# UoB-HPC/stdpar-nbody

Measured on AMD Instinct MI355X. Metric: body-steps/sec + %FP64 peak, 3D double all-pairs N=2^20 at 1/2/4/8 GPUs, higher is better.
Workload: dtype f64

## Files before the change

### stdpar-nbody_amd/csrc/all_pairs.hip

```cpp
#include "common.hpp"

#include <atomic>
#include <cstdlib>
#include <mutex>
#include <type_traits>
#include <vector>

namespace nbody {

constexpr int kBlock = 256;
constexpr int kWaves = kBlock / 64;

struct ap_config {
  int split = 0;
  int tpt   = 0;
  int path  = 0;
};
static std::atomic<uint32_t> g_ap_default{0};

static ap_config ap_config_of(const nbody_state* s) {
  const uint32_t t = s->tuning ? s->tuning : g_ap_default.load(std::memory_order_relaxed);
  ap_config c;
  c.split = int(t & 15u);
  c.tpt   = int((t >> 4) & 3u);
// ... 14 lines not shown
__global__ __launch_bounds__(kBlock) void all_pairs_softened_kernel(const T* __restrict__ m, const T* __restrict__ x,
                                                                    T* __restrict__ a, T c, uint32_t sz, uint32_t first,
                                                                    uint32_t count, T e2) {
  const k1_rule* const rule = nullptr;
#define K1_SOFT true
#include "k1_tile_body.inc"
#undef K1_SOFT
}

template <typename T, int D>
__global__ __launch_bounds__(kBlock) void pack_sources_kernel(const T* __restrict__ m, const T* __restrict__ x,
                                                              src_rec<T, D>* __restrict__ out, uint32_t sz, uint32_t padded) {
  const uint32_t j = blockIdx.x * kBlock + threadIdx.x;
  if (j >= padded) return;
  src_rec<T, D> r;
#pragma unroll
  for (int k = 0; k < 3; ++k) r.p[k] = (k < D && j < sz) ? x[uint64_t(j) * D + (k < D ? k : 0)] : T(0);
  r.m    = j < sz ? m[j] : T(0);
  out[j] = r;
}

template <typename T, int D, bool PACK, bool MOMENTS>
__global__ __launch_bounds__(kBlock) void k1_prepare_kernel(const T* __restrict__ m, const T* __restrict__ x, src_rec<T, D>* __restrict__ out,
                                                            uint32_t sz, uint32_t padded, k1_rule* rule, double* partial,
                                                            uint32_t* turn, uint32_t turn_words) {
  const uint32_t j = blockIdx.x * kBlock + threadIdx.x;
  T p[D];
#pragma unroll
  for (int k = 0; k < D; ++k) p[k] = j < sz ? x[uint64_t(j) * D + k] : T(0);
  if constexpr (PACK) {
    if (j < padded) {
      src_rec<T, D> r;
#pragma unroll
      for (int k = 0; k < 3; ++k) r.p[k] = k < D ? p[k < D ? k : 0] : T(0);
      r.m    = j < sz ? m[j] : T(0);
      out[j] = r;
    }
  }
  __shared__ double red[2 * D][kWaves];
  __shared__ bool last_s;
  const int lane = threadIdx.x & 63, wave = threadIdx.x >> 6;
  if constexpr (MOMENTS) {
    double s1[D], s2[D];
#pragma unroll
    for (int k = 0; k < D; ++k) {
      const double d = j < sz ? double(p[k]) - double(x[k]) : 0.0;
      s1[k] = d;
      s2[k] = d * d;
    }
#pragma unroll
    for (int k = 0; k < D; ++k)
      for (int off = 32; off > 0; off >>= 1) {
        s1[k] += __shfl_xor(s1[k], off, 64);
        s2[k] += __shfl_xor(s2[k], off, 64);
      }
    if (lane == 0) {
#pragma unroll
      for (int k = 0; k < D; ++k) {
        red[k][wave]     = s1[k];
// ... 52 lines not shown
  for (uint32_t w = threadIdx.x; w < turn_words; w += kBlock) turn[w] = 0u;
  if (threadIdx.x == 0) __hip_atomic_store(&rule->ticket, 0u, __ATOMIC_RELAXED, __HIP_MEMORY_SCOPE_AGENT);
}

template <int JS>
constexpr int kSgprWaves = JS > kWaves ? JS : kWaves;

constexpr uint32_t kTurnSpins  = 1u << 26;
constexpr uint32_t kTurnPoison = 0xffffffffu;
struct k1_status {
  uint32_t err, block, group, chunk;
  unsigned long long polls, waits;
};
struct k1_handoff {
  void* sums;
  uint32_t* turn;
  k1_status* status;
  uint32_t spins;
  uint32_t delay;
  uint32_t late;
};
template <typename T, int D, int R, int JS, int RULE = 0>
__global__ __launch_bounds__(64 * kSgprWaves<JS>) void all_pairs_force_sgpr_kernel(const src_rec<T, D>* __restrict__ packed,
                                                                                   const T* __restrict__ x, T* a, T c, uint32_t sz,
                                                                                   uint32_t first, uint32_t count,
                                                                                   uint32_t tiles_per_chunk, k1_handoff h,
                                                                                   const k1_rule* __restrict__ rule) {
  [[maybe_unused]] constexpr T e2 = T(0);
#define K1_SOFT false
#include "k1_sgpr_body.inc"
#undef K1_SOFT
}
template <typename T, int D, int R, int JS>
__global__ __launch_bounds__(64 * kSgprWaves<JS>) void all_pairs_softened_sgpr_kernel(const src_rec<T, D>* __restrict__ packed,
                                                                                      const T* __restrict__ x, T* a, T c, uint32_t sz,
                                                                                      uint32_t first, uint32_t count,
                                                                                      uint32_t tiles_per_chunk, k1_handoff h, T e2) {
  constexpr int RULE = 0;
  const k1_rule* const rule = nullptr;
#define K1_SOFT true
#include "k1_sgpr_body.inc"
#undef K1_SOFT
}

namespace {
struct scratch_buf {
  void* ptr  = nullptr;
  size_t cap = 0;
};
struct packed_slot {
  int device;
  hipStream_t stream;
  scratch_buf buf[6];
  std::vector<void*> retired;
  bool k1_dirty  = false;
  bool k1_failed = false;
};
std::mutex g_packed_mu;
std::vector<packed_slot> g_packed_slots;
}

int ap_scratch_get(hipStream_t st, int which, size_t bytes, void** out) {
  const int dev = stream_device(st);
  std::lock_guard<std::mutex> lock(g_packed_mu);
  packed_slot* slot = nullptr;
  for (auto& sl : g_packed_slots)
    if (sl.stream == st && sl.device == dev) slot = &sl;
  if (slot && slot->buf[which].cap >= bytes) {
    *out = slot->buf[which].ptr;
    return NBODY_OK;
  }
  hipStreamCaptureStatus cs = hipStreamCaptureStatusNone;
  if (st != nullptr) (void)hipStreamIsCapturing(st, &cs);
  if (cs != hipStreamCaptureStatusNone) {
    set_error("all-pairs: the scratch buffers of this stream must exist before a step is recorded "
              "(call nbody_all_pairs_force once outside nbody_graph_begin/end, or use a context from nbody_create)");
// ... 78 lines not shown
    else p.r = blocks_r2 * uint64_t(p.js) >= 8192 ? 2 : 1;
  }
  *out = p;
  return NBODY_OK;
}

int ap_pack_sources(const nbody_state* s, hipStream_t st, void** packed_out) {
  const uint32_t padded = (s->sz + kTileJ - 1) / kTileJ * kTileJ;
  const size_t tsz      = s->dtype == NBODY_F32 ? 4 : 8;
  void* scratch         = nullptr;
  if (int r = ap_scratch_get(st, 0, 4 * tsz * size_t(padded), &scratch)) return r;
  int rc = dispatch(s->dtype, s->dim, [&](auto tg) {
    using T         = typename decltype(tg)::type;
    constexpr int D = decltype(tg)::dim;
    hipLaunchKernelGGL((pack_sources_kernel<T, D>), dim3((padded + kBlock - 1) / kBlock), dim3(kBlock), 0, st,
                       static_cast<const T*>(s->m), static_cast<const T*>(s->x), static_cast<src_rec<T, D>*>(scratch), s->sz, padded);
    NB_HIP(hipGetLastError());
    return int(NBODY_OK);
  });
  *packed_out = scratch;
  return rc;
}

static size_t ap_rule_bytes(uint32_t sz, int dim) {
  const size_t padded = (size_t(sz) + kTileJ - 1) / kTileJ * kTileJ;
  return 32 + sizeof(double) * 2 * size_t(dim) * (padded / kBlock);
}

template <typename T, int D>
static int ap_prepare(const nbody_state* s, hipStream_t st, bool pack, src_rec<T, D>** packed_out, const k1_rule** rule_out,
                      uint32_t* turn, size_t turn_words, bool with_rule = true) {
  const uint32_t padded = (s->sz + kTileJ - 1) / kTileJ * kTileJ;
  const bool moments    = with_rule && s->sz >= kFarMinBodies;
  void* scratch         = nullptr;
  if (pack)
    if (int r = ap_scratch_get(st, 0, 4 * sizeof(T) * size_t(padded), &scratch)) return r;
  void* q = nullptr;
  if (int r = ap_scratch_get(st, 3, ap_rule_bytes(s->sz, D), &q)) return r;
  auto* rule    = static_cast<k1_rule*>(q);
  auto* partial = reinterpret_cast<double*>(static_cast<char*>(q) + 32);
  auto* out     = static_cast<src_rec<T, D>*>(scratch);
  const dim3 grid(padded / kBlock), block(kBlock);
  const T *m = static_cast<const T*>(s->m), *x = static_cast<const T*>(s->x);
  const uint32_t words = uint32_t(turn_words);
  if (pack && moments) hipLaunchKernelGGL((k1_prepare_kernel<T, D, true, true>), grid, block, 0, st, m, x, out, s->sz, padded, rule, partial, turn, words);
  else if (pack) hipLaunchKernelGGL((k1_prepare_kernel<T, D, true, false>), grid, block, 0, st, m, x, out, s->sz, padded, rule, partial, turn, words);
  else if (moments) hipLaunchKernelGGL((k1_prepare_kernel<T, D, false, true>), grid, block, 0, st, m, x, out, s->sz, padded, rule, partial, turn, words);
  NB_HIP(hipGetLastError());
  if (packed_out) *packed_out = out;
  *rule_out = moments ? rule : nullptr;
  return NBODY_OK;
}

constexpr uint32_t kCollectMaxBlocks = 2048;
static bool k1_collect(uint32_t target_blocks, uint32_t chunks) {
  uint32_t limit = kCollectMaxBlocks;
  if (const char* e = experiment_env("NBODY_K1_COLLECT_MAX")) limit = uint32_t(atoi(e));
  return chunks > 1 && uint64_t(target_blocks) * chunks <= limit;
}
template <typename T, int D, int R, int JS>
static size_t k1_collect_bytes(uint32_t target_blocks, uint32_t chunks) {
  constexpr int TG = kSgprWaves<JS> / JS;
  return sizeof(T) * size_t(chunks) * target_blocks * TG * R * D * 64;
}

template <int R, int JS>
static size_t sgpr_turn_words(uint32_t count) {
  constexpr int TG = kSgprWaves<JS> / JS, TB = TG * 64 * R;
  return size_t((count + TB - 1) / TB) * TG;
}

template <typename T, int D, int R, int JS, bool SOFT>
static int launch_all_pairs_sgpr(const nbody_state* s, const k1_plan& plan, hipStream_t st, T e2) {
  constexpr int TB = (kSgprWaves<JS> / JS) * 64 * R;
  uint32_t blocks  = (s->count + TB - 1) / TB;
  if (blocks == 0) return NBODY_OK;
  k1_handoff h{nullptr, nullptr, nullptr, kTurnSpins, 0u, 0u};
  if (plan.chunks > 1) {
    void* q = nullptr;
    if (int r = ap_scratch_get(st, 1, sizeof(uint32_t) * sgpr_turn_words<R, JS>(s->count), &q)) return r;
    h.turn = static_cast<uint32_t*>(q);
    if (k1_collect(blocks, plan.chunks)) {
      if (int r = ap_scratch_get(st, 5, k1_collect_bytes<T, D, R, JS>(blocks, plan.chunks), &q)) return r;
      h.sums = q;
    }
    if (int r = ap_scratch_get(st, 4, sizeof(k1_status), &q)) return r;
    h.status = static_cast<k1_status*>(q);
    if (const char* e = experiment_env("NBODY_K1_TURN_SPINS")) h.spins = uint32_t(strtoul(e, nullptr, 10));
    if (const char* e = experiment_env("NBODY_K1_HANDOFF_DELAY")) h.delay = uint32_t(strtoul(e, nullptr, 10));
    if (const char* e = experiment_env("NBODY_K1_HANDOFF_LATE")) h.late = uint32_t(strtoul(e, nullptr, 10));
    if (const char* e = experiment_env("NBODY_K1_NO_HANDOFF"); e && e[0] == '1') h.turn = nullptr, h.sums = nullptr;
    if (const char* e = experiment_env("NBODY_K1_COLLECT"); e && e[0] == '0') h.sums = nullptr;
  }
  src_rec<T, D>* packed = nullptr;
  const k1_rule* rule   = nullptr;
  if (int r = ap_prepare<T, D>(s, st, true, &packed, &rule, h.turn, h.turn ? sgpr_turn_words<R, JS>(s->count) : 0, !SOFT)) return r;
  if constexpr (SOFT) {
    hipLaunchKernelGGL((all_pairs_softened_sgpr_kernel<T, D, R, JS>), dim3(blocks, plan.chunks), dim3(64 * kSgprWaves<JS>), 0, st,
                       packed, static_cast<const T*>(s->x), static_cast<T*>(s->a), static_cast<T>(s->c), s->sz, s->first, s->count,
                       plan.tiles_per_chunk, h, e2);
    NB_HIP(hipGetLastError());
    if (h.turn != nullptr && h.sums == nullptr) ap_status_mark(st);
    return NBODY_OK;
  }
#ifdef NBODY_EXPERIMENTS
  if (const char* e = getenv("NBODY_K1_RULE_FORCE"); e && JS == 8 && D == 3) {
    if (e[0] == '1')
      hipLaunchKernelGGL((all_pairs_force_sgpr_kernel<T, D, R, JS, 1>), dim3(blocks, plan.chunks), dim3(64 * kSgprWaves<JS>), 0, st,
                         packed, static_cast<const T*>(s->x), static_cast<T*>(s->a), static_cast<T>(s->c), s->sz, s->first, s->count,
                         plan.tiles_per_chunk, h, rule);
    else
      hipLaunchKernelGGL((all_pairs_force_sgpr_kernel<T, D, R, JS, 2>), dim3(blocks, plan.chunks), dim3(64 * kSgprWaves<JS>), 0, st,
                         packed, static_cast<const T*>(s->x), static_cast<T*>(s->a), static_cast<T>(s->c), s->sz, s->first, s->count,
                         plan.tiles_per_chunk, h, rule);
    NB_HIP(hipGetLastError());
    return NBODY_OK;
  }
#endif
  hipLaunchKernelGGL((all_pairs_force_sgpr_kernel<T, D, R, JS>), dim3(blocks, plan.chunks), dim3(64 * kSgprWaves<JS>), 0, st,
                     packed, static_cast<const T*>(s->x), static_cast<T*>(s->a), static_cast<T>(s->c), s->sz, s->first, s->count,
                     plan.tiles_per_chunk, h, rule);
  NB_HIP(hipGetLastError());
  if (h.turn != nullptr && h.sums == nullptr) ap_status_mark(st);
  return NBODY_OK;
}

template <typename T, int D, int R, int JS, bool SOFT>
static int launch_all_pairs(const nbody_state* s, hipStream_t st, T e2) {
  constexpr int TB = (kWaves / JS) * 64 * R;
  uint32_t blocks  = (s->count + TB - 1) / TB;
  if (blocks == 0) return NBODY_OK;
  if constexpr (SOFT) {
    hipLaunchKernelGGL((all_pairs_softened_kernel<T, D, R, JS>), dim3(blocks), dim3(kBlock), 0, st, static_cast<const T*>(s->m),
                       static_cast<const T*>(s->x), static_cast<T*>(s->a), static_cast<T>(s->c), s->sz, s->first, s->count, e2);
    NB_HIP(hipGetLastError());
    return NBODY_OK;
  }
  const k1_rule* rule = nullptr;
  if (int r = ap_prepare<T, D>(s, st, false, nullptr, &rule, nullptr, 0)) return r;
  hipLaunchKernelGGL((all_pairs_force_kernel<T, D, R, JS>), dim3(blocks), dim3(kBlock), 0, st, static_cast<const T*>(s->m),
                     static_cast<const T*>(s->x), static_cast<T*>(s->a), static_cast<T>(s->c), s->sz, s->first, s->count, rule);
  NB_HIP(hipGetLastError());
  return NBODY_OK;
}

template <typename F>
static bool with_k1_instance(const k1_plan& p, F&& fn) {
#define NB_CASE(RR, JJ)                                                                       \
  if (p.r == RR && p.js == JJ) {                                                              \
    fn(std::integral_constant<int, RR>{}, std::integral_constant<int, JJ>{});                 \
    return true;                                                                              \
  }
  NB_CASE(1, 1);
  NB_CASE(1, 2);
  NB_CASE(1, 4);
  NB_CASE(2, 1);
  NB_CASE(2, 2);
  NB_CASE(2, 4);
  if (p.scalar) {
    NB_CASE(1, 8);
    NB_CASE(2, 8);
  }
// ... 4 lines not shown
template <typename T, int D, bool SOFT = false>
static int all_pairs_dispatch(const nbody_state* s, hipStream_t st, T e2 = T(0)) {
  k1_plan p;
  if (int rc = plan_all_pairs<T>(s, &p)) return rc;
  int rc = NBODY_OK;
  const bool found = with_k1_instance(p, [&](auto r, auto js) {
    constexpr int R = decltype(r)::value, JS = decltype(js)::value;
    rc = p.scalar ? launch_all_pairs_sgpr<T, D, R, JS, SOFT>(s, p, st, e2)
                  : (JS <= kWaves ? launch_all_pairs<T, D, R, (JS <= kWaves ? JS : 1), SOFT>(s, st, e2) : int(NBODY_ERR_ARG));
  });
  if (!found) {
    set_error("all-pairs: unsupported config split=%d targets_per_thread=%d", p.js, p.r);
    return NBODY_ERR_ARG;
  }
  return rc;
}

template <typename T, int D>
static int all_pairs_describe(const nbody_state* s, char* out, size_t len) {
  k1_plan p;
  if (int rc = plan_all_pairs<T>(s, &p)) return rc;
  const char* t = sizeof(T) == 8 ? "double" : "float";
  const char* pair = sizeof(T) == 4 ? (s->sz >= kFarMinBodies ? "rsq+rcp[m y^3 at r2 >= 4 if sparse]" : "rsq+rcp")
                                    : s->sz >= kFarMinBodies ? "far3[-eps if sparse]/near3" : "far3/near3";
  if (p.scalar) {
    bool collect = false;
    with_k1_instance(p, [&](auto r, auto js) {
      constexpr int TB = (kSgprWaves<decltype(js)::value> / decltype(js)::value) * 64 * decltype(r)::value;
      collect = k1_collect((s->count + TB - 1) / TB, p.chunks);
    });
    snprintf(out, len, "all_pairs_force_sgpr_kernel<%s,%d,R=%d,JS=%d> tile=%d chunks=%u%s pair=%s", t, D, p.r, p.js, kTileJ, p.chunks,
             p.chunks > 1 ? (collect ? "(summed in chunk order by the last to arrive)" : "(summed in turn into a)") : "", pair);
  }
  else
    snprintf(out, len, "all_pairs_force_kernel<%s,%d,R=%d,JS=%d> tile=%d chunks=1 pair=%s", t, D, p.r, p.js, kTileJ, pair);
  return NBODY_OK;
}

int ap_scratch_reserve(hipStream_t st, const nbody_state* s) {
  void* q             = nullptr;
  const size_t tsz    = s->dtype == NBODY_F32 ? 4 : 8;
  const size_t padded = (size_t(s->sz) + 2 * kTileJ - 1) / (2 * kTileJ) * (2 * kTileJ);
  if (int r = ap_scratch_get(st, 0, 4 * tsz * padded, &q)) return r;
  if (int r = ap_scratch_get(st, 3, ap_rule_bytes(s->sz, s->dim), &q)) return r;
  return dispatch(s->dtype, s->dim, [&](auto tg) {
    using T = typename decltype(tg)::type;
    k1_plan p;
    if (int rc = plan_all_pairs<T>(s, &p)) return rc;
    if (!p.scalar || p.chunks <= 1) return int(NBODY_OK);
    size_t words = 0;
    with_k1_instance(p, [&](auto r, auto js) { words = sgpr_turn_words<decltype(r)::value, decltype(js)::value>(s->count); });
    if (!words) return int(NBODY_OK);
    if (int rc = ap_scratch_get(st, 1, sizeof(uint32_t) * words, &q)) return rc;
    size_t sums = 0;
    with_k1_instance(p, [&](auto r, auto js) {
      constexpr int RR = decltype(r)::value, JJ = decltype(js)::value;
      const uint32_t blocks = (s->count + (kSgprWaves<JJ> / JJ) * 64 * RR - 1) / ((kSgprWaves<JJ> / JJ) * 64 * RR);
      if (k1_collect(blocks, p.chunks)) sums = k1_collect_bytes<T, decltype(tg)::dim, RR, JJ>(blocks, p.chunks);
    });
    if (sums)
      if (int rc = ap_scratch_get(st, 5, sums, &q)) return rc;
    return ap_scratch_get(st, 4, sizeof(k1_status), &q);
  });
}

void ap_status_mark(hipStream_t st) {
// ... 590 lines not shown
  }
  return NBODY_OK;
}

extern "C" int nbody_all_pairs_describe(const nbody_state* s, char* out, size_t len) {
  NB_ARG(out != nullptr && len > 0, "out is NULL");
  if (int r = check_state(s)) return r;
  return dispatch(s->dtype, s->dim, [&](auto tg) {
    using TG = decltype(tg);
    return all_pairs_describe<typename TG::type, TG::dim>(s, out, len);
  });
}

extern "C" int nbody_all_pairs_pair_rule(const nbody_state* s, void* stream, int* sparse_out, double* volume_out) {
  NB_ARG(sparse_out != nullptr, "sparse_out is NULL");
  if (int r = check_state(s)) return r;
  device_guard guard(stream_device(as_stream(stream)));
  *sparse_out = 0;
  if (volume_out) *volume_out = 0.0;
  return dispatch(s->dtype, s->dim, [&](auto tg) {
    using T         = typename decltype(tg)::type;
    constexpr int D = decltype(tg)::dim;
    const k1_rule* rule = nullptr;
    if (int r = ap_prepare<T, D>(s, as_stream(stream), false, nullptr, &rule, nullptr, 0)) return r;
    if (rule == nullptr) return int(NBODY_OK);
    k1_rule host;
    NB_HIP(hipMemcpyAsync(&host, rule, sizeof host, hipMemcpyDeviceToHost, as_stream(stream)));
    NB_HIP(hipStreamSynchronize(as_stream(stream)));
    *sparse_out = host.sparse ? 1 : 0;
    if (volume_out) *volume_out = host.volume;
    return int(NBODY_OK);
  });
}

extern "C" int nbody_all_pairs_force(const nbody_state* s, void* stream) {
  if (int r = check_state(s)) return r;
  device_guard guard(stream_device(as_stream(stream)));
  return dispatch(s->dtype, s->dim, [&](auto tg) {
    using TG = decltype(tg);
    return all_pairs_dispatch<typename TG::type, TG::dim>(s, as_stream(stream));
  });
}

extern "C" int nbody_all_pairs_softened_force(const nbody_state* s, double eps, void* stream) {
  if (int r = check_state(s)) return r;
  return dispatch(s->dtype, s->dim, [&](auto tg) {
    using TG = decltype(tg);
// ... 35 lines not shown
```

### stdpar-nbody_amd/csrc/common.hpp

```cpp
#pragma once
#include <hip/hip_runtime.h>

#include <cfloat>
#include <cstdarg>
#include <cstdint>
#include <cstdio>
#include <cstdlib>
#include <cstring>

#include "../../include/nbody_hip.h"

namespace nbody {

void set_error(const char* fmt, ...);
int hip_fail(hipError_t e, const char* what, const char* file, int line);

#define NB_HIP(call)                                                                   \
  do {                                                                                 \
    hipError_t e_ = (call);                                                            \
    if (e_ != hipSuccess) return ::nbody::hip_fail(e_, #call, __FILE__, __LINE__);     \
  } while (0)

#define NB_ARG(cond, ...)                \
  do {                                   \
// ... 111 lines not shown
    if constexpr (POLISH >= 3) {
      double q = __builtin_fma(e2, e2, e2);
      return __builtin_fma(zm, q, zm);
    } else {
      return __builtin_fma(zm, e2, zm);
    }
  }

  static constexpr uint32_t near_hi = 0x3EF00000u;
  static constexpr uint32_t far_hi = 0x40100000u;
  template <bool EPS = true>
  __device__ static __forceinline__ double weight_far(double r2, double mj, double k15, double k1875, double eps = DBL_EPSILON) {
    double y  = __builtin_amdgcn_rsq(r2);
    double a  = y * y;
    double e  = __builtin_fma(-r2, a, 1.0);
    double y3 = a * y;
    double p  = __builtin_fma(e, k1875, k15);
    double g;
    if constexpr (EPS) g = __builtin_fma(p, e, -(eps * y3));
    else g = p * e;
    double my = mj * y3;
    return __builtin_fma(my, g, my);
  }
};

template <>
struct pair_math<float> {
  static constexpr float tiny = 1e-37f;
  __device__ static __forceinline__ float weight(float r2, float mj) {
    float y0 = __builtin_amdgcn_rsqf(r2);
    float d3 = __builtin_fmaf(r2, r2 * y0, FLT_EPSILON);
    return __builtin_amdgcn_rcpf(d3) * mj;
  }
  static constexpr uint32_t far_bits = 0x40800000u;
};

template <typename T, int D>
struct alignas(sizeof(T) * 4) src_rec {
  T p[3];
  T m;
};

template <typename T, int D>
__device__ __forceinline__ void pair_accumulate(T (&acc)[D], const T (&xi)[D], const src_rec<T, D>& s) {
  T d[D];
#pragma unroll
  for (int k = 0; k < D; ++k) d[k] = s.p[k] - xi[k];
  T r2 = pair_math<T>::tiny;
#pragma unroll
  for (int k = 0; k < D; ++k) r2 = __builtin_elementwise_fma(d[k], d[k], r2);
  T w = pair_math<T>::weight(r2, s.m);
#pragma unroll
  for (int k = 0; k < D; ++k) acc[k] = __builtin_elementwise_fma(w, d[k], acc[k]);
}

template <typename T, int D, int NB>
__device__ __forceinline__ void pair_accumulate_multi(T (&acc)[D], const T (&xi)[D], const src_rec<T, D>* s) {
  T d[NB][D], r2[NB], w[NB];
#pragma unroll
  for (int b = 0; b < NB; ++b) {
#pragma unroll
    for (int k = 0; k < D; ++k) d[b][k] = s[b].p[k] - xi[k];
  }
#pragma unroll
  for (int b = 0; b < NB; ++b) {
// ... 25 lines not shown
#pragma unroll
    for (int k = 0; k < D; ++k) r2[b] = __builtin_elementwise_fma(d[b][k], d[b][k], r2[b]);
  }
#pragma unroll
  for (int b = 0; b < NB; ++b) {
    w[b]              = pair_math<double>::weight_far(r2[b], s[b].m, k15, k1875);
    const uint32_t hi = uint32_t(__builtin_bit_cast(unsigned long long, r2[b]) >> 32);
    lowest            = hi < lowest ? hi : lowest;
  }
#pragma unroll
  for (int b = 0; b < NB; ++b) {
#pragma unroll
    for (int k = 0; k < D; ++k) acc[k] = __builtin_elementwise_fma(w[b], d[b][k], acc[k]);
  }
}

template <typename T>
struct pair_consts {
  __device__ __forceinline__ pair_consts() {}
};
template <>
struct pair_consts<double> {
  double k15, k1875;
  __device__ __forceinline__ pair_consts() : k15(1.5), k1875(1.875) {
    asm volatile("" : "+v"(k15));
    asm volatile("" : "+s"(k1875));
  }
};

template <typename T, int D, int R, int U, bool ffar>
__device__ __forceinline__ void pair_batch(T (&acc)[R][D], const T (&xi)[R][D], const src_rec<T, D> (&s)[U],
                                           const pair_consts<T>& pc) {
  if constexpr (sizeof(T) == 4) {
    if constexpr (!ffar) {
#pragma unroll
      for (int u = 0; u < U; ++u)
#pragma unroll
        for (int r = 0; r < R; ++r) pair_accumulate<T, D>(acc[r], xi[r], s[u]);
    } else {
      T d[U][R][D], r2[U][R], w[U][R];
      uint32_t lowest = 0xffffffffu;
#pragma unroll
      for (int u = 0; u < U; ++u)
#pragma unroll
        for (int r = 0; r < R; ++r) {
#pragma unroll
          for (int k = 0; k < D; ++k) d[u][r][k] = s[u].p[k] - xi[r][k];
          T q = pair_math<T>::tiny;
#pragma unroll
          for (int k = 0; k < D; ++k) q = __builtin_elementwise_fma(d[u][r][k], d[u][r][k], q);
          r2[u][r]            = q;
          const uint32_t bits = __builtin_bit_cast(uint32_t, q);
          lowest              = bits < lowest ? bits : lowest;
        }
      T y[U][R];
// ... 21 lines not shown
#pragma unroll
          for (int k = 0; k < D; ++k) acc[r][k] = __builtin_elementwise_fma(w[u][r], d[u][r][k], acc[r][k]);
    }
  } else {
    T d[U][R][D], r2[U][R], w[U][R];
    uint32_t lowest = 0xffffffffu;
#pragma unroll
    for (int u = 0; u < U; ++u)
#pragma unroll
      for (int r = 0; r < R; ++r) {
#pragma unroll
        for (int k = 0; k < D; ++k) d[u][r][k] = s[u].p[k] - xi[r][k];
        T q = pair_math<T>::tiny;
#pragma unroll
        for (int k = 0; k < D; ++k) q = __builtin_elementwise_fma(d[u][r][k], d[u][r][k], q);
        r2[u][r] = q;
        const uint32_t hi = uint32_t(__builtin_bit_cast(unsigned long long, q) >> 32);
        lowest            = hi < lowest ? hi : lowest;
      }
    if constexpr (!ffar) {
#pragma unroll
      for (int u = 0; u < U; ++u)
#pragma unroll
        for (int r = 0; r < R; ++r) w[u][r] = pair_math<T>::template weight_far<true>(r2[u][r], s[u].m, pc.k15, pc.k1875);
      if (__builtin_expect(__builtin_amdgcn_ballot_w64(lowest < pair_math<T>::near_hi) != 0ull, 0)) {
#pragma unroll
        for (int u = 0; u < U; ++u)
#pragma unroll
          for (int r = 0; r < R; ++r) {
            const uint32_t hi = uint32_t(__builtin_bit_cast(unsigned long long, r2[u][r]) >> 32);
            const T wn        = pair_math<T>::template weight<3>(r2[u][r], s[u].m);
            w[u][r]           = hi < pair_math<T>::near_hi ? wn : w[u][r];
          }
      }
    } else if (__builtin_expect(__builtin_amdgcn_ballot_w64(lowest < pair_math<T>::far_hi) == 0ull, 1)) {
#pragma unroll
      for (int u = 0; u < U; ++u)
#pragma unroll
        for (int r = 0; r < R; ++r) w[u][r] = pair_math<T>::template weight_far<false>(r2[u][r], s[u].m, pc.k15, pc.k1875);
    } else {
#pragma unroll
      for (int u = 0; u < U; ++u)
#pragma unroll
        for (int r = 0; r < R; ++r) {
          const uint32_t hi  = uint32_t(__builtin_bit_cast(unsigned long long, r2[u][r]) >> 32);
          const uint32_t ehi = hi < pair_math<T>::far_hi ? 0x3CB00000u : 0u;
          const T eps        = __builtin_bit_cast(T, (unsigned long long)ehi << 32);
          w[u][r]            = pair_math<T>::template weight_far<true>(r2[u][r], s[u].m, pc.k15, pc.k1875, eps);
        }
      if (__builtin_expect(__builtin_amdgcn_ballot_w64(lowest < pair_math<T>::near_hi) != 0ull, 0)) {
#pragma unroll
        for (int u = 0; u < U; ++u)
#pragma unroll
          for (int r = 0; r < R; ++r) {
            const uint32_t hi = uint32_t(__builtin_bit_cast(unsigned long long, r2[u][r]) >> 32);
            const T wn        = pair_math<T>::template weight<3>(r2[u][r], s[u].m);
            w[u][r]           = hi < pair_math<T>::near_hi ? wn : w[u][r];
          }
      }
    }
#pragma unroll
    for (int u = 0; u < U; ++u)
#pragma unroll
      for (int r = 0; r < R; ++r)
#pragma unroll
        for (int k = 0; k < D; ++k) acc[r][k] = __builtin_elementwise_fma(w[u][r], d[u][r][k], acc[r][k]);
  }
}

template <typename T>
__device__ __forceinline__ T soft_weight(T q, T mj, const pair_consts<T>& pc) {
  if constexpr (sizeof(T) == 8) {
    return pair_math<double>::template weight_far<false>(q, mj, pc.k15, pc.k1875);
  } else {
    const T y = __builtin_amdgcn_rsqf(q);
    return mj * ((y * y) * y);
  }
}

template <typename T, int D, int R, int U>
__device__ __forceinline__ void pair_batch_soft(T (&acc)[R][D], const T (&xi)[R][D], const src_rec<T, D> (&s)[U],
                                                const pair_consts<T>& pc, T e2) {
  T d[U][R][D], q[U][R], w[U][R];
#pragma unroll
  for (int u = 0; u < U; ++u)
#pragma unroll
    for (int r = 0; r < R; ++r) {
#pragma unroll
      for (int k = 0; k < D; ++k) d[u][r][k] = s[u].p[k] - xi[r][k];
      T t = e2;
#pragma unroll
      for (int k = 0; k < D; ++k) t = __builtin_elementwise_fma(d[u][r][k], d[u][r][k], t);
      q[u][r] = t;
    }
#pragma unroll
  for (int u = 0; u < U; ++u)
#pragma unroll
    for (int r = 0; r < R; ++r) w[u][r] = soft_weight<T>(q[u][r], s[u].m, pc);
#pragma unroll
  for (int u = 0; u < U; ++u)
#pragma unroll
    for (int r = 0; r < R; ++r)
#pragma unroll
      for (int k = 0; k < D; ++k) acc[r][k] = __builtin_elementwise_fma(w[u][r], d[u][r][k], acc[r][k]);
}

template <typename T>
constexpr T kSoftMinE2 = sizeof(T) == 4 ? T(0x1p-84f) : T(0x1p-680);

template <typename T>
inline int check_softening(double eps, T* e2_out) {
  NB_ARG(eps > 0.0 && eps <= DBL_MAX, "softening length eps = %g must be finite and > 0", eps);
  const T te = T(eps);
  const T e2 = te * te;
  NB_ARG(e2 >= kSoftMinE2<T> && e2 <= (sizeof(T) == 4 ? T(FLT_MAX) : T(DBL_MAX)),
         "softening length eps = %g: eps^2 = %g in %s is outside [%g, max]: its square must be a normal number whose ^(-3/2) is finite",
         eps, double(e2), sizeof(T) == 4 ? "float" : "double", double(kSoftMinE2<T>));
  *e2_out = e2;
  return NBODY_OK;
}

// ... 6 lines not shown
};
constexpr uint32_t kFarMinBodies = 32768;
template <int D>
constexpr double kFarMinVolume = D == 3 ? 1.7e5 : 6.4e4;
__device__ __forceinline__ bool ap_far_mode(const k1_rule* __restrict__ rule) {
  if (rule == nullptr) return false;
  return __builtin_amdgcn_readfirstlane(int(rule->sparse)) != 0;
}

constexpr int kTileJ = 512;

typedef uint32_t sgpr16 __attribute__((ext_vector_type(16)));
template <typename V>
__device__ __forceinline__ sgpr16 sload16(const void* p, V& tie) {
  sgpr16 r;
  asm volatile("s_load_dwordx16 %0, %2, 0x0" : "=s"(r), "+v"(tie) : "s"(p));
  return r;
}
template <typename V>
__device__ __forceinline__ void swait(sgpr16& v, V& tie) {
  asm volatile("s_waitcnt lgkmcnt(0)" : "+s"(v), "+v"(tie));
}

inline int check_tuning(int split, int tpt, int path) {
  NB_ARG(split == 0 || split == 1 || split == 2 || split == 4 || split == 8, "split must be 0, 1, 2, 4 or 8 (got %d)", split);
  NB_ARG(tpt >= 0 && tpt <= 2, "targets_per_thread must be 0, 1 or 2 (got %d)", tpt);
  NB_ARG(path >= 0 && path <= 2, "source path must be 0 (auto), 1 (LDS tiles) or 2 (scalar stream), got %d", path);
  return NBODY_OK;
}

int ap_scratch_reserve(hipStream_t st, const nbody_state* view);
void ap_scratch_release(hipStream_t st);
int ap_scratch_get(hipStream_t st, int which, size_t bytes, void** out);
void ap_status_mark(hipStream_t st);
int ap_status_read(hipStream_t st, unsigned long long out[6], bool clear);
int ap_pack_sources(const nbody_state* s, hipStream_t st, void** packed_out);
void ap_auto_chunks(uint32_t sz, uint32_t* chunks, uint32_t* tiles_per_chunk);
int energies_from_sums(const nbody_state* s, hipStream_t st, int (*fill)(void* sums, void* ctx), void* ctx, void* ke_out, void* pe_out);

}
```

### stdpar-nbody_amd/csrc/k1_sgpr_body.inc

```
  using rec_t = src_rec<T, D>;
  constexpr int TG  = kSgprWaves<JS> / JS;
  constexpr int TB  = TG * 64 * R;
  constexpr int SUB = kTileJ / JS;
  __shared__ T partial[(JS > 1) ? (JS - 1) * TG * 64 * R * D : 1];
  const int lane   = threadIdx.x & 63;
  const int wave   = __builtin_amdgcn_readfirstlane(threadIdx.x >> 6);
  const int tgroup = wave / JS;
  const int jpart  = wave % JS;
  T xi[R][D], acc[R][D];
  uint32_t ti[R];
#pragma unroll
  for (int r = 0; r < R; ++r) {
    uint32_t local = blockIdx.x * TB + tgroup * (64 * R) + r * 64 + lane;
    ti[r]          = local;
    uint64_t i     = uint64_t(first) + (local < count ? local : 0u);
#pragma unroll
    for (int k = 0; k < D; ++k) {
      xi[r][k]  = x[i * D + k];
      acc[r][k] = T(0);
    }
  }
  const uint32_t ntiles = (sz + kTileJ - 1) / kTileJ;
  const uint32_t t0     = blockIdx.y * tiles_per_chunk;
  const uint32_t t1     = min(ntiles, t0 + tiles_per_chunk);
  const pair_consts<T> pc;
  const bool ffar       = !K1_SOFT && ap_far_mode(rule);
  const uint32_t nsteps = (t1 - t0) * SUB;
  constexpr int U = 64 / int(sizeof(rec_t));
  struct batch_t {
    rec_t r[U];
  };
  auto batch = [&](uint32_t k) { return packed + (uint64_t(t0 + k / SUB) * kTileJ + uint32_t(jpart) * SUB + (k % SUB)); };
  auto run = [&](auto ff) {
    constexpr bool FF = decltype(ff)::value;
    sgpr16 A = sload16(batch(0), xi[0][0]), B;
    for (uint32_t k = 0; k < nsteps; k += 2 * U) {
      swait(A, acc[0][0]);
      B = sload16(batch(k + U), xi[0][0]);
      {
        const batch_t ba = __builtin_bit_cast(batch_t, A);
        if constexpr (K1_SOFT) pair_batch_soft<T, D, R, U>(acc, xi, ba.r, pc, e2);
        else pair_batch<T, D, R, U, FF>(acc, xi, ba.r, pc);
      }
      swait(B, acc[0][0]);
      A = sload16(batch(k + 2 * U < nsteps ? k + 2 * U : k), xi[0][0]);
      {
        const batch_t bb = __builtin_bit_cast(batch_t, B);
        if constexpr (K1_SOFT) pair_batch_soft<T, D, R, U>(acc, xi, bb.r, pc, e2);
        else pair_batch<T, D, R, U, FF>(acc, xi, bb.r, pc);
      }
    }
    swait(A, acc[0][0]);
  };
  if constexpr (K1_SOFT) run(std::false_type{});
  else if constexpr (RULE == 1) run(std::false_type{});
  else if constexpr (RULE == 2) run(std::true_type{});
  else if (ffar) run(std::true_type{});
  else run(std::false_type{});
  if constexpr (JS > 1) {
    if (jpart > 0) {
#pragma unroll
      for (int r = 0; r < R; ++r)
#pragma unroll
        for (int k = 0; k < D; ++k) partial[((((jpart - 1) * TG + tgroup) * R + r) * D + k) * 64 + lane] = acc[r][k];
    }
    __syncthreads();
    if (jpart == 0) {
#pragma unroll
      for (int p = 1; p < JS; ++p)
#pragma unroll
        for (int r = 0; r < R; ++r)
#pragma unroll
          for (int k = 0; k < D; ++k) acc[r][k] += partial[((((p - 1) * TG + tgroup) * R + r) * D + k) * 64 + lane];
    }
  }
// ... 118 lines not shown
```

### stdpar-nbody_amd/csrc/k1_tile_body.inc

```
  using rec_t = src_rec<T, D>;
  constexpr int TG  = kWaves / JS;
  constexpr int TB  = TG * 64 * R;
  constexpr int LPT = kTileJ / kBlock;
  constexpr int SUB = kTileJ / JS;

  __shared__ rec_t tile[kTileJ];
  __shared__ T partial[(JS > 1) ? (JS - 1) * TG * 64 * R * D : 1];

  const int lane   = threadIdx.x & 63;
  const int wave   = threadIdx.x >> 6;
  const int tgroup = wave / JS;
  const int jpart  = wave % JS;

  T xi[R][D], acc[R][D];
  uint32_t ti[R];
#pragma unroll
  for (int r = 0; r < R; ++r) {
    uint32_t local = blockIdx.x * TB + tgroup * (64 * R) + r * 64 + lane;
    ti[r]          = local;
    uint64_t i     = uint64_t(first) + (local < count ? local : 0u);
#pragma unroll
    for (int k = 0; k < D; ++k) {
      xi[r][k]  = x[i * D + k];
      acc[r][k] = T(0);
// ... 17 lines not shown
#pragma unroll
        for (int k = 0; k < D; ++k) stage[q].p[k] = T(0);
        stage[q].m = T(0);
      }
      if (D == 2) stage[q].p[2] = T(0);
    }
  };

  stage_load(0);
  auto run = [&](auto ff) {
    constexpr bool FF = decltype(ff)::value;
    for (uint32_t t = 0; t < ntiles; ++t) {
      __syncthreads();
#pragma unroll
      for (int q = 0; q < LPT; ++q) tile[q * kBlock + threadIdx.x] = stage[q];
      __syncthreads();
      if (t + 1 < ntiles) stage_load(t + 1);

      const rec_t* src = &tile[jpart * SUB];
      constexpr int U  = 64 / int(sizeof(rec_t));
#pragma unroll 2
      for (int jj = 0; jj < SUB; jj += U) {
        rec_t s[U];
#pragma unroll
        for (int u = 0; u < U; ++u) s[u] = src[jj + u];
        if constexpr (K1_SOFT) pair_batch_soft<T, D, R, U>(acc, xi, s, pc, e2);
        else pair_batch<T, D, R, U, FF>(acc, xi, s, pc);
      }
    }
  };
  if constexpr (K1_SOFT) run(std::false_type{});
  else if (ffar) run(std::true_type{});
  else run(std::false_type{});

  if constexpr (JS > 1) {
    __syncthreads();
    if (jpart > 0) {
#pragma unroll
      for (int r = 0; r < R; ++r)
#pragma unroll
        for (int k = 0; k < D; ++k) partial[((((jpart - 1) * TG + tgroup) * R + r) * D + k) * 64 + lane] = acc[r][k];
    }
    __syncthreads();
    if (jpart == 0) {
#pragma unroll
      for (int p = 1; p < JS; ++p)
#pragma unroll
        for (int r = 0; r < R; ++r)
#pragma unroll
          for (int k = 0; k < D; ++k) acc[r][k] += partial[((((p - 1) * TG + tgroup) * R + r) * D + k) * 64 + lane];
// ... 12 lines not shown
```

Measured before the change: 1.739 million.

## Precompute per-source 1.5m and 1.875m constants to fold the far-field weight polynomial

The f64 prepare kernel now writes per-source constants 1.5*m and 1.875*m into a new scratch buffer. The SGPR force kernel streams these alongside the packed sources, splitting them across a vector global load and a scalar load. It then uses a folded weight formula (t = fma(e, m1875, m15); s = fma(t, e, m)) that drops the per-pair multiplies by mass. This cuts FP64 VALU ops per interaction, at the cost of extra memory traffic, extra scratch, and a more complex load/wait pipeline that adds VGPR pressure.

```diff
diff --git a/stdpar-nbody_amd/csrc/all_pairs.hip b/stdpar-nbody_amd/csrc/all_pairs.hip
--- a/stdpar-nbody_amd/csrc/all_pairs.hip
+++ b/stdpar-nbody_amd/csrc/all_pairs.hip
@@ -60,7 +60,7 @@
 
 template <typename T, int D, bool PACK, bool MOMENTS>
 __global__ __launch_bounds__(kBlock) void k1_prepare_kernel(const T* __restrict__ m, const T* __restrict__ x, src_rec<T, D>* __restrict__ out,
-                                                            uint32_t sz, uint32_t padded, k1_rule* rule, double* partial,
+                                                            cst_batch* __restrict__ cst, uint32_t sz, uint32_t padded, k1_rule* rule, double* partial,
                                                             uint32_t* turn, uint32_t turn_words) {
   const uint32_t j = blockIdx.x * kBlock + threadIdx.x;
   T p[D];
@@ -73,6 +73,11 @@
       for (int k = 0; k < 3; ++k) r.p[k] = k < D ? p[k < D ? k : 0] : T(0);
       r.m    = j < sz ? m[j] : T(0);
       out[j] = r;
+      if constexpr (sizeof(T) == 8) {
+        const src_cst<T> k  = src_cst<T>::of(r.m);
+        cst[j / 2].m15[j % 2]   = k.m15;
+        cst[j / 2].m1875[j % 2] = k.m1875;
+      }
     }
   }
   __shared__ double red[2 * D][kWaves];
@@ -171,6 +176,7 @@
 };
 template <typename T, int D, int R, int JS, int RULE = 0>
 __global__ __launch_bounds__(64 * kSgprWaves<JS>) void all_pairs_force_sgpr_kernel(const src_rec<T, D>* __restrict__ packed,
+                                                                                   const cst_batch* __restrict__ cst,
                                                                                    const T* __restrict__ x, T* a, T c, uint32_t sz,
                                                                                    uint32_t first, uint32_t count,
                                                                                    uint32_t tiles_per_chunk, k1_handoff h,
@@ -182,6 +188,7 @@
 }
 template <typename T, int D, int R, int JS>
 __global__ __launch_bounds__(64 * kSgprWaves<JS>) void all_pairs_softened_sgpr_kernel(const src_rec<T, D>* __restrict__ packed,
+                                                                                      const cst_batch* __restrict__ cst,
                                                                                       const T* __restrict__ x, T* a, T c, uint32_t sz,
                                                                                       uint32_t first, uint32_t count,
                                                                                       uint32_t tiles_per_chunk, k1_handoff h, T e2) {
@@ -200,7 +207,7 @@
 struct packed_slot {
   int device;
   hipStream_t stream;
-  scratch_buf buf[6];
+  scratch_buf buf[7];
   std::vector<void*> retired;
   bool k1_dirty  = false;
   bool k1_failed = false;
@@ -325,32 +332,40 @@
   return rc;
 }
 
+static size_t ap_cst_bytes(size_t padded) { return sizeof(cst_batch) * (padded / 2); }
+
 static size_t ap_rule_bytes(uint32_t sz, int dim) {
   const size_t padded = (size_t(sz) + kTileJ - 1) / kTileJ * kTileJ;
   return 32 + sizeof(double) * 2 * size_t(dim) * (padded / kBlock);
 }
 
 template <typename T, int D>
-static int ap_prepare(const nbody_state* s, hipStream_t st, bool pack, src_rec<T, D>** packed_out, const k1_rule** rule_out,
-                      uint32_t* turn, size_t turn_words, bool with_rule = true) {
+static int ap_prepare(const nbody_state* s, hipStream_t st, bool pack, src_rec<T, D>** packed_out, const cst_batch** cst_out,
+                      const k1_rule** rule_out, uint32_t* turn, size_t turn_words, bool with_rule = true) {
   const uint32_t padded = (s->sz + kTileJ - 1) / kTileJ * kTileJ;
   const bool moments    = with_rule && s->sz >= kFarMinBodies;
   void* scratch         = nullptr;
-  if (pack)
+  void* consts          = nullptr;
+  if (pack) {
     if (int r = ap_scratch_get(st, 0, 4 * sizeof(T) * size_t(padded), &scratch)) return r;
+    if (sizeof(T) == 8)
+      if (int r = ap_scratch_get(st, 6, ap_cst_bytes(padded), &consts)) return r;
+  }
   void* q = nullptr;
   if (int r = ap_scratch_get(st, 3, ap_rule_bytes(s->sz, D), &q)) return r;
   auto* rule    = static_cast<k1_rule*>(q);
   auto* partial = reinterpret_cast<double*>(static_cast<char*>(q) + 32);
   auto* out     = static_cast<src_rec<T, D>*>(scratch);
+  auto* cst     = static_cast<cst_batch*>(consts);
   const dim3 grid(padded / kBlock), block(kBlock);
   const T *m = static_cast<const T*>(s->m), *x = static_cast<const T*>(s->x);
   const uint32_t words = uint32_t(turn_words);
-  if (pack && moments) hipLaunchKernelGGL((k1_prepare_kernel<T, D, true, true>), grid, block, 0, st, m, x, out, s->sz, padded, rule, partial, turn, words);
-  else if (pack) hipLaunchKernelGGL((k1_prepare_kernel<T, D, true, false>), grid, block, 0, st, m, x, out, s->sz, padded, rule, partial, turn, words);
-  else if (moments) hipLaunchKernelGGL((k1_prepare_kernel<T, D, false, true>), grid, block, 0, st, m, x, out, s->sz, padded, rule, partial, turn, words);
+  if (pack && moments) hipLaunchKernelGGL((k1_prepare_kernel<T, D, true, true>), grid, block, 0, st, m, x, out, cst, s->sz, padded, rule, partial, turn, words);
+  else if (pack) hipLaunchKernelGGL((k1_prepare_kernel<T, D, true, false>), grid, block, 0, st, m, x, out, cst, s->sz, padded, rule, partial, turn, words);
+  else if (moments) hipLaunchKernelGGL((k1_prepare_kernel<T, D, false, true>), grid, block, 0, st, m, x, out, cst, s->sz, padded, rule, partial, turn, words);
   NB_HIP(hipGetLastError());
   if (packed_out) *packed_out = out;
+  if (cst_out) *cst_out = cst;
   *rule_out = moments ? rule : nullptr;
   return NBODY_OK;
 }
@@ -396,11 +411,12 @@
     if (const char* e = experiment_env("NBODY_K1_COLLECT"); e && e[0] == '0') h.sums = nullptr;
   }
   src_rec<T, D>* packed = nullptr;
+  const cst_batch* cst  = nullptr;
   const k1_rule* rule   = nullptr;
-  if (int r = ap_prepare<T, D>(s, st, true, &packed, &rule, h.turn, h.turn ? sgpr_turn_words<R, JS>(s->count) : 0, !SOFT)) return r;
+  if (int r = ap_prepare<T, D>(s, st, true, &packed, &cst, &rule, h.turn, h.turn ? sgpr_turn_words<R, JS>(s->count) : 0, !SOFT)) return r;
   if constexpr (SOFT) {
     hipLaunchKernelGGL((all_pairs_softened_sgpr_kernel<T, D, R, JS>), dim3(blocks, plan.chunks), dim3(64 * kSgprWaves<JS>), 0, st,
-                       packed, static_cast<const T*>(s->x), static_cast<T*>(s->a), static_cast<T>(s->c), s->sz, s->first, s->count,
+                       packed, cst, static_cast<const T*>(s->x), static_cast<T*>(s->a), static_cast<T>(s->c), s->sz, s->first, s->count,
                        plan.tiles_per_chunk, h, e2);
     NB_HIP(hipGetLastError());
     if (h.turn != nullptr && h.sums == nullptr) ap_status_mark(st);
@@ -410,18 +426,18 @@
   if (const char* e = getenv("NBODY_K1_RULE_FORCE"); e && JS == 8 && D == 3) {
     if (e[0] == '1')
       hipLaunchKernelGGL((all_pairs_force_sgpr_kernel<T, D, R, JS, 1>), dim3(blocks, plan.chunks), dim3(64 * kSgprWaves<JS>), 0, st,
-                         packed, static_cast<const T*>(s->x), static_cast<T*>(s->a), static_cast<T>(s->c), s->sz, s->first, s->count,
+                         packed, cst, static_cast<const T*>(s->x), static_cast<T*>(s->a), static_cast<T>(s->c), s->sz, s->first, s->count,
                          plan.tiles_per_chunk, h, rule);
     else
       hipLaunchKernelGGL((all_pairs_force_sgpr_kernel<T, D, R, JS, 2>), dim3(blocks, plan.chunks), dim3(64 * kSgprWaves<JS>), 0, st,
-                         packed, static_cast<const T*>(s->x), static_cast<T*>(s->a), static_cast<T>(s->c), s->sz, s->first, s->count,
+                         packed, cst, static_cast<const T*>(s->x), static_cast<T*>(s->a), static_cast<T>(s->c), s->sz, s->first, s->count,
                          plan.tiles_per_chunk, h, rule);
     NB_HIP(hipGetLastError());
     return NBODY_OK;
   }
 #endif
   hipLaunchKernelGGL((all_pairs_force_sgpr_kernel<T, D, R, JS>), dim3(blocks, plan.chunks), dim3(64 * kSgprWaves<JS>), 0, st,
-                     packed, static_cast<const T*>(s->x), static_cast<T*>(s->a), static_cast<T>(s->c), s->sz, s->first, s->count,
+                     packed, cst, static_cast<const T*>(s->x), static_cast<T*>(s->a), static_cast<T>(s->c), s->sz, s->first, s->count,
                      plan.tiles_per_chunk, h, rule);
   NB_HIP(hipGetLastError());
   if (h.turn != nullptr && h.sums == nullptr) ap_status_mark(st);
@@ -440,7 +456,7 @@
     return NBODY_OK;
   }
   const k1_rule* rule = nullptr;
-  if (int r = ap_prepare<T, D>(s, st, false, nullptr, &rule, nullptr, 0)) return r;
+  if (int r = ap_prepare<T, D>(s, st, false, nullptr, nullptr, &rule, nullptr, 0)) return r;
   hipLaunchKernelGGL((all_pairs_force_kernel<T, D, R, JS>), dim3(blocks), dim3(kBlock), 0, st, static_cast<const T*>(s->m),
                      static_cast<const T*>(s->x), static_cast<T*>(s->a), static_cast<T>(s->c), s->sz, s->first, s->count, rule);
   NB_HIP(hipGetLastError());
@@ -491,7 +507,7 @@
   if (int rc = plan_all_pairs<T>(s, &p)) return rc;
   const char* t = sizeof(T) == 8 ? "double" : "float";
   const char* pair = sizeof(T) == 4 ? (s->sz >= kFarMinBodies ? "rsq+rcp[m y^3 at r2 >= 4 if sparse]" : "rsq+rcp")
-                                    : s->sz >= kFarMinBodies ? "far3[-eps if sparse]/near3" : "far3/near3";
+                                    : s->sz >= kFarMinBodies ? "far3m[-eps if sparse]/near3" : "far3m/near3";
   if (p.scalar) {
     bool collect = false;
     with_k1_instance(p, [&](auto r, auto js) {
@@ -511,6 +527,8 @@
   const size_t tsz    = s->dtype == NBODY_F32 ? 4 : 8;
   const size_t padded = (size_t(s->sz) + 2 * kTileJ - 1) / (2 * kTileJ) * (2 * kTileJ);
   if (int r = ap_scratch_get(st, 0, 4 * tsz * padded, &q)) return r;
+  if (s->dtype == NBODY_F64)
+    if (int r = ap_scratch_get(st, 6, ap_cst_bytes(padded), &q)) return r;
   if (int r = ap_scratch_get(st, 3, ap_rule_bytes(s->sz, s->dim), &q)) return r;
   return dispatch(s->dtype, s->dim, [&](auto tg) {
     using T = typename decltype(tg)::type;
@@ -1147,7 +1165,7 @@
     using T         = typename decltype(tg)::type;
     constexpr int D = decltype(tg)::dim;
     const k1_rule* rule = nullptr;
-    if (int r = ap_prepare<T, D>(s, as_stream(stream), false, nullptr, &rule, nullptr, 0)) return r;
+    if (int r = ap_prepare<T, D>(s, as_stream(stream), false, nullptr, nullptr, &rule, nullptr, 0)) return r;
     if (rule == nullptr) return int(NBODY_OK);
     k1_rule host;
     NB_HIP(hipMemcpyAsync(&host, rule, sizeof host, hipMemcpyDeviceToHost, as_stream(stream)));
diff --git a/stdpar-nbody_amd/csrc/common.hpp b/stdpar-nbody_amd/csrc/common.hpp
--- a/stdpar-nbody_amd/csrc/common.hpp
+++ b/stdpar-nbody_amd/csrc/common.hpp
@@ -157,6 +157,21 @@
     double my = mj * y3;
     return __builtin_fma(my, g, my);
   }
+
+  static constexpr double eps23 = 2.0 / 3.0 * DBL_EPSILON;
+  template <bool EPS, bool SMASS = false>
+  __device__ static __forceinline__ double weight_far_folded(double r2, double mj, double m15, double m1875, double keps = eps23) {
+    double y  = __builtin_amdgcn_rsq(r2);
+    double a  = y * y;
+    double e  = __builtin_fma(-r2, a, 1.0);
+    double y3 = a * y;
+    if constexpr (EPS) e = __builtin_fma(-keps, y3, e);
+    double t = __builtin_fma(e, m1875, m15);
+    double s;
+    if constexpr (SMASS) asm("v_fma_f64 %0, %1, %2, %3" : "=v"(s) : "v"(t), "v"(e), "s"(mj));
+    else s = __builtin_fma(t, e, mj);
+    return y3 * s;
+  }
 };
 
 template <>
@@ -176,6 +191,19 @@
   T m;
 };
 
+template <typename T>
+struct src_cst {
+  __device__ __forceinline__ static src_cst of(T) { return {}; }
+};
+template <>
+struct src_cst<double> {
+  double m15, m1875;
+  __device__ __forceinline__ static src_cst of(double m) { return {1.5 * m, 1.875 * m}; }
+};
+struct alignas(32) cst_batch {
+  double m15[2], m1875[2];
+};
+
 template <typename T, int D>
 __device__ __forceinline__ void pair_accumulate(T (&acc)[D], const T (&xi)[D], const src_rec<T, D>& s) {
   T d[D];
@@ -247,15 +275,17 @@
 template <>
 struct pair_consts<double> {
   double k15, k1875;
-  __device__ __forceinline__ pair_consts() : k15(1.5), k1875(1.875) {
+  double keps;
+  __device__ __forceinline__ pair_consts() : k15(1.5), k1875(1.875), keps(pair_math<double>::eps23) {
     asm volatile("" : "+v"(k15));
     asm volatile("" : "+s"(k1875));
+    asm("" : "+s"(keps));
   }
 };
 
 template <typename T, int D, int R, int U, bool ffar>
 __device__ __forceinline__ void pair_batch(T (&acc)[R][D], const T (&xi)[R][D], const src_rec<T, D> (&s)[U],
-                                           const pair_consts<T>& pc) {
+                                           const src_cst<T> (&kc)[U], const pair_consts<T>& pc) {
   if constexpr (sizeof(T) == 4) {
     if constexpr (!ffar) {
 #pragma unroll
@@ -323,7 +353,8 @@
 #pragma unroll
       for (int u = 0; u < U; ++u)
 #pragma unroll
-        for (int r = 0; r < R; ++r) w[u][r] = pair_math<T>::template weight_far<true>(r2[u][r], s[u].m, pc.k15, pc.k1875);
+        for (int r = 0; r < R; ++r)
+          w[u][r] = pair_math<T>::template weight_far_folded<true>(r2[u][r], s[u].m, kc[u].m15, kc[u].m1875, pc.keps);
       if (__builtin_expect(__builtin_amdgcn_ballot_w64(lowest < pair_math<T>::near_hi) != 0ull, 0)) {
 #pragma unroll
         for (int u = 0; u < U; ++u)
@@ -338,16 +369,15 @@
 #pragma unroll
       for (int u = 0; u < U; ++u)
 #pragma unroll
-        for (int r = 0; r < R; ++r) w[u][r] = pair_math<T>::template weight_far<false>(r2[u][r], s[u].m, pc.k15, pc.k1875);
+        for (int r = 0; r < R; ++r) w[u][r] = pair_math<T>::template weight_far_folded<false>(r2[u][r], s[u].m, kc[u].m15, kc[u].m1875);
     } else {
 #pragma unroll
       for (int u = 0; u < U; ++u)
 #pragma unroll
         for (int r = 0; r < R; ++r) {
-          const uint32_t hi  = uint32_t(__builtin_bit_cast(unsigned long long, r2[u][r]) >> 32);
-          const uint32_t ehi = hi < pair_math<T>::far_hi ? 0x3CB00000u : 0u;
-          const T eps        = __builtin_bit_cast(T, (unsigned long long)ehi << 32);
-          w[u][r]            = pair_math<T>::template weight_far<true>(r2[u][r], s[u].m, pc.k15, pc.k1875, eps);
+          const uint32_t hi = uint32_t(__builtin_bit_cast(unsigned long long, r2[u][r]) >> 32);
+          const T mine      = hi < pair_math<T>::far_hi ? pc.keps : T(0);
+          w[u][r]           = pair_math<T>::template weight_far_folded<true>(r2[u][r], s[u].m, kc[u].m15, kc[u].m1875, mine);
         }
       if (__builtin_expect(__builtin_amdgcn_ballot_w64(lowest < pair_math<T>::near_hi) != 0ull, 0)) {
 #pragma unroll
@@ -369,6 +399,13 @@
   }
 }
 
+template <typename T, int D, int R, int U, bool ffar>
+__device__ __forceinline__ void pair_batch(T (&acc)[R][D], const T (&xi)[R][D], const src_rec<T, D> (&s)[U], const pair_consts<T>& pc) {
+  static_assert(sizeof(T) == 4, "f64 callers pass the sources' constants (src_cst)");
+  const src_cst<T> none[U] = {};
+  pair_batch<T, D, R, U, ffar>(acc, xi, s, none, pc);
+}
+
 template <typename T>
 __device__ __forceinline__ T soft_weight(T q, T mj, const pair_consts<T>& pc) {
   if constexpr (sizeof(T) == 8) {
@@ -379,9 +416,9 @@
   }
 }
 
-template <typename T, int D, int R, int U>
+template <typename T, int D, int R, int U, bool SSRC = false>
 __device__ __forceinline__ void pair_batch_soft(T (&acc)[R][D], const T (&xi)[R][D], const src_rec<T, D> (&s)[U],
-                                                const pair_consts<T>& pc, T e2) {
+                                                const src_cst<T> (&kc)[U], const pair_consts<T>& pc, T e2) {
   T d[U][R][D], q[U][R], w[U][R];
 #pragma unroll
   for (int u = 0; u < U; ++u)
@@ -397,7 +434,11 @@
 #pragma unroll
   for (int u = 0; u < U; ++u)
 #pragma unroll
-    for (int r = 0; r < R; ++r) w[u][r] = soft_weight<T>(q[u][r], s[u].m, pc);
+    for (int r = 0; r < R; ++r) {
+      if constexpr (sizeof(T) == 8)
+        w[u][r] = pair_math<T>::template weight_far_folded<false, SSRC && R == 1>(q[u][r], s[u].m, kc[u].m15, kc[u].m1875);
+      else w[u][r] = soft_weight<T>(q[u][r], s[u].m, pc);
+    }
 #pragma unroll
   for (int u = 0; u < U; ++u)
 #pragma unroll
@@ -450,6 +491,29 @@
   asm volatile("s_waitcnt lgkmcnt(0)" : "+s"(v), "+v"(tie));
 }
 
+typedef uint32_t reg4 __attribute__((ext_vector_type(4)));
+struct cst_regs {
+  reg4 v, s;
+};
+template <typename V>
+__device__ __forceinline__ cst_regs cload(const void* p, uint32_t vzero, V& tie) {
+  cst_regs r;
+  asm volatile("global_load_dwordx4 %0, %3, %4\n\ts_load_dwordx4 %1, %4, 0x10" : "=&v"(r.v), "=&s"(r.s), "+v"(tie) : "v"(vzero), "s"(p));
+  return r;
+}
+template <typename V>
+__device__ __forceinline__ void cswait(sgpr16& v, cst_regs& c, V& tie) {
+  asm volatile("s_waitcnt vmcnt(0) lgkmcnt(0)" : "+s"(v), "+v"(c.v), "+s"(c.s), "+v"(tie));
+}
+__device__ __forceinline__ void cst_unpack(const cst_regs& c, src_cst<double> (&kc)[2]) {
+  struct pair_t {
+    double d[2];
+  };
+  const pair_t v = __builtin_bit_cast(pair_t, c.v), s = __builtin_bit_cast(pair_t, c.s);
+  kc[0] = {v.d[0], s.d[0]};
+  kc[1] = {v.d[1], s.d[1]};
+}
+
 inline int check_tuning(int split, int tpt, int path) {
   NB_ARG(split == 0 || split == 1 || split == 2 || split == 4 || split == 8, "split must be 0, 1, 2, 4 or 8 (got %d)", split);
   NB_ARG(tpt >= 0 && tpt <= 2, "targets_per_thread must be 0, 1 or 2 (got %d)", tpt);
diff --git a/stdpar-nbody_amd/csrc/k1_sgpr_body.inc b/stdpar-nbody_amd/csrc/k1_sgpr_body.inc
--- a/stdpar-nbody_amd/csrc/k1_sgpr_body.inc
+++ b/stdpar-nbody_amd/csrc/k1_sgpr_body.inc
@@ -31,26 +31,45 @@
     rec_t r[U];
   };
   auto batch = [&](uint32_t k) { return packed + (uint64_t(t0 + k / SUB) * kTileJ + uint32_t(jpart) * SUB + (k % SUB)); };
+  constexpr bool CST = sizeof(T) == 8;
+  auto cbatch = [&](uint32_t k) { return cst + (uint64_t(t0 + k / SUB) * kTileJ + uint32_t(jpart) * SUB + (k % SUB)) / U; };
+  [[maybe_unused]] uint32_t vzero = 0;
+  if constexpr (CST) {
+    asm volatile("" : "+v"(vzero));
+#pragma unroll
+    for (int r = 0; r < R; ++r)
+#pragma unroll
+      for (int k = 0; k < D; ++k) asm volatile("" : "+v"(xi[r][k]));
+  }
   auto run = [&](auto ff) {
     constexpr bool FF = decltype(ff)::value;
-    sgpr16 A = sload16(batch(0), xi[0][0]), B;
+    sgpr16 A, B;
+    [[maybe_unused]] cst_regs CA, CB;
+    auto request = [&](sgpr16& S, cst_regs& C, uint32_t k) {
+      if constexpr (CST) C = cload(cbatch(k), vzero, xi[0][0]);
+      S = sload16(batch(k), xi[0][0]);
+    };
+    auto wait = [&](sgpr16& S, cst_regs& C) {
+      if constexpr (CST) cswait(S, C, acc[0][0]);
+      else swait(S, acc[0][0]);
+    };
+    auto consume = [&](const sgpr16& S, const cst_regs& C) {
+      const batch_t b = __builtin_bit_cast(batch_t, S);
+      src_cst<T> kc[U];
+      if constexpr (CST) cst_unpack(C, kc);
+      if constexpr (K1_SOFT) pair_batch_soft<T, D, R, U, true>(acc, xi, b.r, kc, pc, e2);
+      else pair_batch<T, D, R, U, FF>(acc, xi, b.r, kc, pc);
+    };
+    request(A, CA, 0);
     for (uint32_t k = 0; k < nsteps; k += 2 * U) {
-      swait(A, acc[0][0]);
-      B = sload16(batch(k + U), xi[0][0]);
-      {
-        const batch_t ba = __builtin_bit_cast(batch_t, A);
-        if constexpr (K1_SOFT) pair_batch_soft<T, D, R, U>(acc, xi, ba.r, pc, e2);
-        else pair_batch<T, D, R, U, FF>(acc, xi, ba.r, pc);
-      }
-      swait(B, acc[0][0]);
-      A = sload16(batch(k + 2 * U < nsteps ? k + 2 * U : k), xi[0][0]);
-      {
-        const batch_t bb = __builtin_bit_cast(batch_t, B);
-        if constexpr (K1_SOFT) pair_batch_soft<T, D, R, U>(acc, xi, bb.r, pc, e2);
-        else pair_batch<T, D, R, U, FF>(acc, xi, bb.r, pc);
-      }
-    }
-    swait(A, acc[0][0]);
+      wait(A, CA);
+      request(B, CB, k + U);
+      consume(A, CA);
+      wait(B, CB);
+      request(A, CA, k + 2 * U < nsteps ? k + 2 * U : k);
+      consume(B, CB);
+    }
+    wait(A, CA);
   };
   if constexpr (K1_SOFT) run(std::false_type{});
   else if constexpr (RULE == 1) run(std::false_type{});
diff --git a/stdpar-nbody_amd/csrc/k1_tile_body.inc b/stdpar-nbody_amd/csrc/k1_tile_body.inc
--- a/stdpar-nbody_amd/csrc/k1_tile_body.inc
+++ b/stdpar-nbody_amd/csrc/k1_tile_body.inc
@@ -63,10 +63,14 @@
 #pragma unroll 2
       for (int jj = 0; jj < SUB; jj += U) {
         rec_t s[U];
+        src_cst<T> kc[U];
 #pragma unroll
-        for (int u = 0; u < U; ++u) s[u] = src[jj + u];
-        if constexpr (K1_SOFT) pair_batch_soft<T, D, R, U>(acc, xi, s, pc, e2);
-        else pair_batch<T, D, R, U, FF>(acc, xi, s, pc);
+        for (int u = 0; u < U; ++u) {
+          s[u]  = src[jj + u];
+          kc[u] = src_cst<T>::of(s[u].m);
+        }
+        if constexpr (K1_SOFT) pair_batch_soft<T, D, R, U>(acc, xi, s, kc, pc, e2);
+        else pair_batch<T, D, R, U, FF>(acc, xi, s, kc, pc);
       }
     }
   };
```

Measured after the change: 1.788 million (median of 6 runs). 1.03x the previous value.
